# agent-charon/MinGraph-UNet

Hardware: AMD Instinct MI355X
Metric: segmented Mpix/sec, full MinGraph-UNet forward (U-Net + patch-graph GAT), 512x512 batch (higher is better)
Workload: dtype f32

## Files before the change

mingraph-unet_amd/csrc/common.h:

```cpp
#pragma once
#include <hip/hip_runtime.h>
#include <stdint.h>

namespace mgu {

struct Tuning {
  bool first_mfma = true;
  bool use_halo = true;
  bool halo_tps3 = true;
  int halo_max_ppb = 16;
  bool use_wino = true;
  int wino_mode = -1;
  int wino_prec = 1;
  bool wino_cp_narrow = true;
  bool wino_yfast = false;
  bool convt_frag = true;
  bool wino_deep = true;
  bool wino_cp = true;
  int wino_rounds = 1;
  int wino_ppb_cap = 32;
  bool wgrad_halo = true;
  bool wino_wgrad = true;
  bool convt_dgrad_x3 = true;
  bool wgrad_x3 = true;
  bool wgrad_thin = true;
  bool wino_dgrad = true;
  bool gat_fused = true;
  bool wino_ures = true;
  bool wino_prio = false;
  bool wino_asm_narrow = true;
  int wino_asm = 1;
};
const Tuning& default_tuning();
hipError_t ensure_dyn_lds(const void* func, size_t bytes, bool (&done)[64]);

struct IgemmDesc {
  const Tuning* tn;
  const float* in;
  const float* w;
  const float* wu;
  const float* scale;
  const float* shift;
  float* out;
  int M;
  int H, W;
  int Cp;
  int ldin;
  int KS;
  int K;
  int Kp;
  int N;
  int ldout;
  int coff;
  int relu;
  int out_mode;
  int ct_cout;
  int Hout, Wout;
  float* pool;
  int ldpool;
  double* stat_slots;
  int split_n;
  float* out2;
  int ld2;
};

inline const Tuning& tun(const IgemmDesc& d) { return d.tn ? *d.tn : default_tuning(); }
hipError_t launch_igemm_f32(const IgemmDesc& d, hipStream_t s);
int wino_grid_blocks(const IgemmDesc& d);
bool halo_pool_fusable(const IgemmDesc& d, int dtype);
hipError_t launch_igemm_bf16(const IgemmDesc& d, hipStream_t s);
const char* igemm_kernel_name(const IgemmDesc& d, int dtype);
size_t convt_x3_floats(int Cin, int Cout);
hipError_t launch_pack_convt_x3(const float* w, float* Wx, int Cin, int Cout, hipStream_t s);
bool convt_x3_applicable(const IgemmDesc& d);
hipError_t launch_convt_x3(const IgemmDesc& d, hipStream_t s);
size_t convt_bf16f_floats(int Cin, int Cout);
hipError_t launch_pack_convt_bf16f(const float* w, float* Wf, int Cin, int Cout, hipStream_t s);
bool convt_bf16f_applicable(const IgemmDesc& d);
hipError_t launch_convt_bf16f(const IgemmDesc& d, hipStream_t s);
size_t convt_x3_dgrad_floats(int Cin, int Cout);
hipError_t launch_pack_convt_x3_dgrad(const float* w, float* Wx, int Cin, int Cout, hipStream_t s);
bool convt_x3_dgrad_applicable(const IgemmDesc& d);
hipError_t launch_convt_x3_dgrad(const IgemmDesc& d, hipStream_t s);
hipError_t launch_pack_first_w(const float* w, float* wf, int Cout, int Cin, hipStream_t s);
size_t first_mfma_floats();
bool first_mfma_applicable(int dtype, int Cin, int Cp, int Cout, int ldout, int coff, int64_t H, int64_t W);
hipError_t launch_pack_first_mfma(const float* w, float* wfm, int Cout, int Cin, hipStream_t s);
hipError_t launch_first_mfma(int dtype, const void* in, const float* wfm, const float* scale, const float* shift, void* out, int B, int H,
                             int W, int ldout, int coff, int relu, hipStream_t s);
hipError_t launch_first_mfma_direct(int dtype, const float* x, int64_t sn, int64_t sc, int64_t sh, int64_t sw, int cin, const float* wfm,
                                    const float* scale, const float* shift, void* out, int B, int H, int W, int ldout, int coff, int relu,
                                    hipStream_t s);
bool first_conv_applicable(int dtype, int Cin, int Cp, int Cout, int ldout, int coff);
hipError_t launch_first_conv(int dtype, const void* in, const float* wf, const float* scale, const float* shift, void* out, int B, int H, int W,
                             int Cin, int Cout, int ldout, int coff, int relu, hipStream_t s);
size_t wino_u_floats(int Cout, int Cp);
hipError_t launch_pack_wino_w(const float* w, float* U, int Cout, int Cin, int Cp, int dgrad, int prec, hipStream_t s);
enum { PACK_WINO = 0, PACK_FIRST_W = 1, PACK_CONVT_X3 = 2, PACK_BIAS_TILE = 3, PACK_DGRAD_W = 4, PACK_FIRST_MFMA = 5 };
struct WinoPackItem {
  const float* w;
  float* U;
  int Cout, Cin, Cp, Np, dgrad;
  unsigned blk0;
  int kind;
  int reserved;
};
static_assert(sizeof(WinoPackItem) == 48, "WinoPackItem must have no padding");
constexpr int WINO_PACK_MAX = 64;
struct WinoPackBatch {
  int n, prec;
  unsigned total_blocks;
  WinoPackItem it[WINO_PACK_MAX];
};
bool wino_pack_batch_prepare(WinoPackBatch& b);
hipError_t launch_pack_wino_w_multi(const WinoPackBatch* batch_dev, unsigned total_blocks, hipStream_t s);
bool wino_applicable(const IgemmDesc& d);
hipError_t launch_wino_f32(const IgemmDesc& d, hipStream_t s);
bool wino_asm_applicable(const IgemmDesc& d);
hipError_t launch_wino_cp_asm(const IgemmDesc& d, hipStream_t s);

struct WgradDesc {
  const Tuning* tn;
  const float* z;
  int ldz, zoff;
  const float* in;
  int ldin, inoff, Cp;
  int KS;
  int M, H, W;
  int Hs, Ws;
  int N, K, Kp;
  float* dw;
  size_t dw_capacity;
  int groups;
  int rows_per_split;
};
inline const Tuning& tun(const WgradDesc& d) { return d.tn ? *d.tn : default_tuning(); }
hipError_t launch_wgrad_f32(WgradDesc& d, hipStream_t s);
bool wino_wgrad_applicable(const WgradDesc& d);
hipError_t launch_wino_wgrad_f32(WgradDesc& d, hipStream_t s);
bool wgrad_thin_applicable(const WgradDesc& d);
hipError_t launch_wgrad_thin(WgradDesc& d, hipStream_t s);

constexpr int STAT_ROWS = 576;
constexpr int CHAN_REDUCE_ROWS = 512;
size_t chan_reduce_work_bytes(int Cmax);
hipError_t launch_bn_stats(const float* z, int ldz, int64_t M, int C, double* work, double* sums, hipStream_t s);
hipError_t launch_bn_finalize(const double* sum, const double* sumsq, int64_t M, float eps, float momentum,
                              const float* gamma, const float* beta, float* mean, float* invstd, float* scale,
                              float* shift, float* run_mean, float* run_var, int C, hipStream_t s);
hipError_t launch_bn_finalize_slots(double* slots, int nrows, double* sums, int64_t M, float eps, float momentum, const float* gamma,
                                    const float* beta, float* mean, float* invstd, float* scale, float* shift, float* run_mean,
                                    float* run_var, int C, hipStream_t s);
hipError_t launch_bn_apply_relu(const float* z, const float* scale, const float* shift, float* y, int ldy, int64_t M, int C,
                                hipStream_t s);
hipError_t launch_bn_apply_relu_pool(const float* z, const float* scale, const float* shift, float* y, int ldy, float* pooled, int B, int H,
                                     int W, int C, hipStream_t s);
hipError_t launch_bn_bwd_reduce(const float* dy, int lddy, const float* fwd_scale, const float* fwd_shift, const float* z, int ldz,
                                const float* mean, const float* invstd, int64_t M, int C, double* work, double* sums,
                                float* dbeta, float* dgamma, hipStream_t s);
hipError_t launch_bn_bwd_apply(const float* dy, int lddy, const float* fwd_scale, const float* fwd_shift, const float* z, const float* mean,
                               const float* invstd, const float* gamma, const double* sums, int64_t M, int C, float* dz,
                               double* work, float* dbias, hipStream_t s);
hipError_t launch_bn_bwd_apply_deferred(const float* dy, int lddy, const float* fsc, const float* fsh, const float* z, const float* mean,
                                        const float* invstd, const float* gamma, const double* sums, int64_t M, int C, float* dz,
                                        double* work, int* rows, hipStream_t s);
hipError_t launch_colsum(const float* z, int ldz, int64_t M, int C, double* work, float* out, hipStream_t s);
hipError_t launch_maxpool2_bwd_add(const float* y, int ldy, const float* dpool, float* dskip, int ldd, int B, int H, int W,
                                   int C, hipStream_t s);
hipError_t launch_zero_pad_region(float* buf, int ld, int coff, int C, int B, int H, int W, int h2, int w2, hipStream_t s);
hipError_t launch_ce(const float* logits, const int64_t* labels, int64_t M, int C, long long ignore_index, float grad_scale,
                     float* dlogits, int ldd, double* acc, int* err_word, float* loss_out, hipStream_t s);
hipError_t launch_pack_dgrad_w(const float* w, float* wp, int Cout, int Cin, int Cop, int KS, int Kp, hipStream_t s);
hipError_t launch_pack_convt_dgrad_w(const float* w, float* wp, int Cin, int Cout, int Kp, hipStream_t s);
hipError_t launch_unpack_conv_grad(const float* dwp, int groups, size_t panel_stride, float* g, int Cout, int Cin, int Cp, int KS,
                                   int Kp, hipStream_t s, double* fold_slots = nullptr, int fold_rows = 0, int fold_n = 0, float* fold_out = nullptr);
hipError_t launch_unpack_convt_grad(const float* dwp, int groups, size_t panel_stride, float* g, int Cin, int Cout, int Kp, hipStream_t s);
hipError_t launch_sgd(float* p, const float* g, float* buf, int64_t n, float lr, float momentum, float wd, int step, float grad_scale,
                      hipStream_t s);
hipError_t launch_adam(float* p, const float* g, float* m, float* v, int64_t n, float lr, float b1, float b2, float eps,
                       float wd, int step, float grad_scale, hipStream_t s);

hipError_t launch_pack_input(const float* x, void* out, int dtype, int B, int C, int Cp, int H, int W, int64_t sn, int64_t sc,
                             int64_t sh, int64_t sw, hipStream_t s);
hipError_t launch_maxpool2(const void* in, int ldin, void* out, int dtype, int B, int H, int W, int C, hipStream_t s);
bool patch_mean_head_fusable(int dtype, int C, int ncls);
hipError_t launch_patch_mean(const void* feat, int dtype, float* out, int B, int H, int W, int C, int patch, hipStream_t s,
                             const float* head_w = nullptr, const float* head_b = nullptr, float* logits = nullptr, int ncls = 0);
hipError_t launch_pack_conv_w(const float* w_oihw, void* wp, int dtype, int Cout, int Cin, int Cp, int KS, int Kp, hipStream_t s);
hipError_t launch_pack_convt_w(const float* w_iohw, void* wp, int dtype, int Cin, int Cout, int Kp, hipStream_t s);
hipError_t launch_bn_fold(const float* bias, const float* gamma, const float* beta, const float* mean, const float* var,
                          float eps, float* scale, float* shift, int C, hipStream_t s);
hipError_t launch_bias_tile(const float* bias, float* shift, int C, int reps, hipStream_t s);
hipError_t launch_conv1x1_head(const void* in, int dtype, int ldin, int C, const float* w, const float* bias, float* out,
                               int ldout, int ncls, int64_t npix, hipStream_t s);
hipError_t launch_argmax(const float* logits, int64_t npix, int C, int64_t* pred, hipStream_t s);

hipError_t launch_gat_wa_rows(const float* W, const float* a, float* panel, int row0, int heads, int Fh, int Fin, int Kp, hipStream_t s);
bool gat_fused_applicable(int Fin, int heads, int Fh, int64_t E);
size_t gat_fused_scratch_floats(int Fin, int heads, int Fh);
hipError_t launch_gat_prep(const float* W, const float* a, float* wa, unsigned* Wx, int heads, int Fh, int Fin, hipStream_t s);
hipError_t launch_gat_stmax(const float* x, const float* wa, int N, int Fin, int heads, const int32_t* rowptr, const int32_t* col,
                            const int32_t* gp, int G, float alpha, float* st, int32_t* node_graph, unsigned long long* gmax, int gstride,
                            unsigned gen, hipStream_t s);
hipError_t launch_gat_fused(const float* x, int Fin, const float* st, const int32_t* rowptr, const int32_t* col, const int32_t* gp, int G,
                            const unsigned long long* gmax, const unsigned* Wx, int N, int heads, int Fh, int concat, float alpha, float* out,
                            int gstride, unsigned gen, hipStream_t s);
hipError_t launch_gat_node_graph(const int32_t* gp, int G, int nodes_per_graph, int N, int32_t* node_graph, hipStream_t s);
hipError_t launch_gat_edge_max(const float* st, const int32_t* rowptr, const int32_t* col, const int32_t* node_graph, int N,
                               int heads, float alpha, unsigned long long* gmax_enc, int gstride, unsigned gen, hipStream_t s);
hipError_t launch_gat_aggregate(const float* wh, int P, const float* st, const int32_t* rowptr, const int32_t* col,
                                const int32_t* node_graph, const unsigned long long* gmax_enc, int N, int64_t E, int heads, int Fh,
                                int concat, float alpha, float* out, int gstride, unsigned gen, hipStream_t s);

}
```

mingraph-unet_amd/csrc/convt_x3.hip:

```cpp
#include <hip/hip_runtime.h>
#include <stdint.h>

#include <algorithm>
#include <type_traits>

#include "common.h"
#include "pack_small.h"

namespace mgu {

typedef float f32x16 __attribute__((ext_vector_type(16)));
typedef float f32x4 __attribute__((ext_vector_type(4)));
typedef unsigned u32x4 __attribute__((ext_vector_type(4)));
typedef __bf16 bf16x8 __attribute__((ext_vector_type(8)));

namespace {

__device__ __forceinline__ void split3_pack(const float a, const float b, unsigned& p0, unsigned& p1, unsigned& p2) {
  const unsigned ua = __float_as_uint(a), ub = __float_as_uint(b);
  p0 = __builtin_amdgcn_perm(ub, ua, 0x07060302u);
  const float ra = a - __uint_as_float(ua & 0xffff0000u), rb = b - __uint_as_float(ub & 0xffff0000u);
  const unsigned va = __float_as_uint(ra), vb = __float_as_uint(rb);
  p1 = __builtin_amdgcn_perm(vb, va, 0x07060302u);
  const float sa = ra - __uint_as_float(va & 0xffff0000u), sb = rb - __uint_as_float(vb & 0xffff0000u);
  p2 = __builtin_amdgcn_perm(__float_as_uint(sb), __float_as_uint(sa), 0x07060302u);
}

__device__ __forceinline__ f32x16 mfma_bf16(const u32x4 a, const u32x4 b, const f32x16 c) {
  return __builtin_amdgcn_mfma_f32_32x32x16_bf16(__builtin_bit_cast(bf16x8, a), __builtin_bit_cast(bf16x8, b), c, 0, 0, 0);
}

__global__ void pack_convt_x3_kernel(const float* __restrict__ w, uint16_t* __restrict__ Wx, int Cin, int Cout) {
  pack_convt_x3_body(w, Wx, Cin, Cout, 0, blockIdx.x, gridDim.x);
}

__device__ __forceinline__ void lds_barrier() { asm volatile("s_waitcnt lgkmcnt(0)\n\ts_barrier" ::: "memory"); }

template <int MODE, int NI>
__global__ __launch_bounds__(256, 2) void convt2x2_x3_kernel(const float* __restrict__ in, const int ldin, const uint16_t* __restrict__ Wx,
                                                             const float* __restrict__ shift, float* __restrict__ out, const int M,
                                                             const int H, const int W, const int Cin, const int Cout, const int ldout,
                                                             const int coff, const int Hout, const int Wout, const int ntn,
                                                             const int nblocks) {
  constexpr int AP = 40, ABUF = 3 * 128 * AP;
  __shared__ __attribute__((aligned(16))) uint16_t As[2 * ABUF];
  __shared__ int rowoff[128];
  const int chunk = gridDim.x >> 3;
  const int lb = (blockIdx.x & 7) * chunk + (blockIdx.x >> 3);
  if (lb >= nblocks) return;
  const int nt = lb % ntn, mt = lb / ntn;
  const int tid = threadIdx.x, lane = tid & 63, wave = tid >> 6;
  const int wm = wave >> 1, wn = wave & 1, lr = lane & 31, lh = lane >> 5;
  const int bm0 = mt * 128;
  const int HW = H * W;
  long long pix0;
  {
    const int img = bm0 / HW, rem = bm0 - img * HW, y = rem / W;
    pix0 = ((long long)img * Hout + 2 * y) * Wout + 2 * (rem - y * W);
  }
  if (tid < 128) {
    const int m = bm0 + tid;
    int off = 0;
    if (m < M) {
      const int img = m / HW, rem = m - img * HW, y = rem / W, x = rem - y * W;
      off = (int)((((long long)img * Hout + 2 * y) * Wout + 2 * x - pix0) * ldout);
    }
    rowoff[tid] = off;
  }

  const int arow = tid >> 3, ach = (tid & 7) * 4;
  const float* aptr[4];
#pragma unroll
  for (int j = 0; j < 4; ++j) {
    const int m = min(bm0 + j * 32 + arow, M - 1);
    if (MODE == 0) {
      aptr[j] = in + (size_t)m * ldin + ach;
    } else {
      const int img = m / HW, rem = m - img * HW, y = rem / W, x = rem - y * W;
      aptr[j] = in + (((size_t)img * Hout + 2 * y) * Wout + 2 * x) * ldin + ach;
    }
  }
  const int nk = (MODE == 0 ? Cin : 4 * Cin) >> 5;
  const int spq = Cin >> 5;
  auto koff = [&](int s) -> int {
    if (MODE == 0) return s * 32;
    const int q = s / spq;
    return ((q >> 1) * Wout + (q & 1)) * ldin + (s - q * spq) * 32;
  };
  f32x4 areg[2][4];
  auto load_a = [&](int s, auto set_t) {
    constexpr int set = decltype(set_t)::value;
    const int ko = koff(s);
#pragma unroll
    for (int j = 0; j < 4; ++j) areg[set][j] = *reinterpret_cast<const f32x4*>(aptr[j] + ko);
  };
  auto store_a = [&](int buf, auto set_t) {
    constexpr int set = decltype(set_t)::value;
    uint16_t* const base = As + buf * ABUF + arow * AP + ach;
#pragma unroll
    for (int j = 0; j < 4; ++j) {
      unsigned p[3][2];
      split3_pack(areg[set][j][0], areg[set][j][1], p[0][0], p[1][0], p[2][0]);
      split3_pack(areg[set][j][2], areg[set][j][3], p[0][1], p[1][1], p[2][1]);
#pragma unroll
      for (int q = 0; q < 3; ++q) *reinterpret_cast<uint2*>(base + (q * 128 + j * 32) * AP) = uint2{p[q][0], p[q][1]};
    }
  };

  const int nt128 = NI == 2 ? nt : nt >> 1, sub0 = NI == 2 ? wn * 2 : (nt & 1) * 2 + wn;
  const u32x4* const bp = reinterpret_cast<const u32x4*>(Wx) + ((size_t)nt128 * (2 * nk) * 12 + sub0 * 3) * 64 + lane;
  u32x4 br[2][3 * NI];
  auto load_b = [&](int kk, auto buf_t) {
    constexpr int buf = decltype(buf_t)::value;
#pragma unroll
    for (int f = 0; f < 3 * NI; ++f) br[buf][f] = bp[((size_t)kk * 12 + f) * 64];
  };

  f32x16 acc[2][NI];
#pragma unroll
  for (int mi = 0; mi < 2; ++mi)
#pragma unroll
    for (int ni = 0; ni < NI; ++ni)
#pragma unroll
      for (int r = 0; r < 16; ++r) acc[mi][ni][r] = 0.f;

  const int aoff = (wm * 64 + lr) * AP + lh * 8;
  auto half_step = [&](int buf, int ss, auto bb_t) {
    constexpr int bb = decltype(bb_t)::value;
    u32x4 pa[2][3];
#pragma unroll
    for (int mi = 0; mi < 2; ++mi)
#pragma unroll
      for (int q = 0; q < 3; ++q)
        pa[mi][q] = *reinterpret_cast<const u32x4*>(As + buf * ABUF + (q * 128 + mi * 32) * AP + aoff + ss * 16);
#pragma unroll
    for (int mi = 0; mi < 2; ++mi)
#pragma unroll
      for (int ni = 0; ni < NI; ++ni) {
        f32x16 t = acc[mi][ni];
        t = mfma_bf16(pa[mi][2], br[bb][ni * 3 + 0], t);
        t = mfma_bf16(pa[mi][0], br[bb][ni * 3 + 2], t);
        t = mfma_bf16(pa[mi][1], br[bb][ni * 3 + 1], t);
        t = mfma_bf16(pa[mi][1], br[bb][ni * 3 + 0], t);
        t = mfma_bf16(pa[mi][0], br[bb][ni * 3 + 1], t);
        t = mfma_bf16(pa[mi][0], br[bb][ni * 3 + 0], t);
        acc[mi][ni] = t;
      }
  };
  using B0 = std::integral_constant<int, 0>;
  using B1 = std::integral_constant<int, 1>;
  const int nkk = 2 * nk;
  load_a(0, B0{});
  load_a(min(1, nk - 1), B1{});
  load_b(0, B0{});
  store_a(0, B0{});
  lds_barrier();
  auto second_half_and_stage = [&](int buf, auto bb_t, auto set_t) {
    half_step(buf, 1, bb_t);
    store_a(buf ^ 1, set_t);
#pragma unroll
    for (int k = 0; k < 12 * NI; ++k) {
      __builtin_amdgcn_sched_group_barrier(0x008, 1, 0);
      __builtin_amdgcn_sched_group_barrier(0x002, NI == 2 ? 4 : 8, 0);
    }
    __builtin_amdgcn_sched_group_barrier(0x200, 12, 0);
  };
  for (int s = 0; s < nk; s += 2) {
    load_a(min(s + 2, nk - 1), B0{});
    load_b(min(2 * s + 1, nkk - 1), B1{});
    __builtin_amdgcn_sched_barrier(0);
    half_step(0, 0, B0{});
    load_b(min(2 * s + 2, nkk - 1), B0{});
    __builtin_amdgcn_sched_barrier(0);
    second_half_and_stage(0, B1{}, B1{});
    __builtin_amdgcn_sched_barrier(0);
    lds_barrier();
    if (s + 1 >= nk) break;
    load_a(min(s + 3, nk - 1), B1{});
    load_b(min(2 * s + 3, nkk - 1), B1{});
    __builtin_amdgcn_sched_barrier(0);
    half_step(1, 0, B0{});
    load_b(min(2 * s + 4, nkk - 1), B0{});
    __builtin_amdgcn_sched_barrier(0);
    second_half_and_stage(1, B1{}, B0{});
    __builtin_amdgcn_sched_barrier(0);
    lds_barrier();
  }

  float* const tile_out = MODE == 0 ? out + (size_t)pix0 * ldout + coff : out + (size_t)bm0 * ldout + coff;
  const bool full_m = bm0 + 128 <= M;
  auto store_tile = [&](auto guarded_t) {
    constexpr bool GUARDED = decltype(guarded_t)::value;
#pragma unroll
    for (int ni = 0; ni < NI; ++ni) {
      const int n = nt * (64 * NI) + wn * (32 * NI) + ni * 32 + lr;
      int ncol = n;
      if (MODE == 0) {
        const int q = n / Cout;
        ncol = ((q >> 1) * Wout + (q & 1)) * ldout + (n - q * Cout);
      }
      const float sh = shift ? shift[n] : 0.f;
#pragma unroll
      for (int mi = 0; mi < 2; ++mi)
#pragma unroll
        for (int r = 0; r < 16; ++r) {
          const int rrow = wm * 64 + mi * 32 + (r & 3) + 8 * (r >> 2) + 4 * lh;
          const unsigned idx = (unsigned)((MODE == 0 ? rowoff[rrow] : rrow * ldout) + ncol);
          const float v = acc[mi][ni][r] + sh;
          if (!GUARDED) tile_out[idx] = v;
          else if (bm0 + rrow < M) tile_out[idx] = v;
        }
    }
  };
#if defined(MGU_DIAG) && MGU_DIAG == 7
  {
    float sacc = 0.f;
#pragma unroll
    for (int mi = 0; mi < 2; ++mi)
#pragma unroll
      for (int ni = 0; ni < NI; ++ni)
#pragma unroll
        for (int r = 0; r < 16; ++r) sacc += acc[mi][ni][r];
    if (sacc == 123.456f) tile_out[tid] = sacc;
  }
#else
  if (full_m) store_tile(std::false_type{});
  else store_tile(std::true_type{});
#endif
}

}

size_t convt_x3_floats(int Cin, int Cout) { return (size_t)Cin * Cout * 6; }


namespace {

__global__ void pack_convt_x3_dgrad_kernel(const float* __restrict__ w, uint16_t* __restrict__ Wx, int Cin, int Cout) {
  pack_convt_x3_body(w, Wx, Cin, Cout, 1, blockIdx.x, gridDim.x);
}

}

size_t convt_x3_dgrad_floats(int Cin, int Cout) { return (size_t)((Cin + 127) / 128 * 128) * Cout * 6; }

hipError_t launch_pack_convt_x3_dgrad(const float* w, float* Wx, int Cin, int Cout, hipStream_t s) {
  if ((Cin & 63) || (Cout & 31)) return hipErrorInvalidValue;
  hipLaunchKernelGGL(pack_convt_x3_dgrad_kernel, dim3((unsigned)std::min<int64_t>(4096, ((int64_t)Cin * Cout * 4 + 255) / 256)), dim3(256), 0, s, w,
                     reinterpret_cast<uint16_t*>(Wx), Cin, Cout);
  return hipGetLastError();
}

bool convt_x3_dgrad_applicable(const IgemmDesc& d) {
  return d.KS == 2 && d.wu && d.out_mode == 0 && (d.Cp & 31) == 0 && d.K == 4 * d.Cp && (d.N & 63) == 0 && (d.ldin & 3) == 0 && !d.scale &&
         !d.shift && !d.relu && !d.split_n && !d.pool && tun(d).wino_prec != 0 && (long)d.M * d.ldout < (1l << 31) &&
         (long)d.Hout * d.Wout * d.ldin < (1l << 31);
}

hipError_t launch_convt_x3_dgrad(const IgemmDesc& d, hipStream_t s) {
  const bool wide = (d.N & 127) == 0;
  const int mtiles = (d.M + 127) / 128, ntn = d.N / (wide ? 128 : 64);
  const int nb = mtiles * ntn;
  const int chunk = (nb + 7) / 8;
  if (wide)
    hipLaunchKernelGGL((convt2x2_x3_kernel<1, 2>), dim3(chunk * 8), dim3(256), 0, s, d.in, d.ldin, reinterpret_cast<const uint16_t*>(d.wu),
                       (const float*)nullptr, d.out, d.M, d.H, d.W, d.Cp, d.N, d.ldout, d.coff, d.Hout, d.Wout, ntn, nb);
  else
    hipLaunchKernelGGL((convt2x2_x3_kernel<1, 1>), dim3(chunk * 8), dim3(256), 0, s, d.in, d.ldin, reinterpret_cast<const uint16_t*>(d.wu),
                       (const float*)nullptr, d.out, d.M, d.H, d.W, d.Cp, d.N, d.ldout, d.coff, d.Hout, d.Wout, ntn, nb);
  return hipGetLastError();
}

hipError_t launch_pack_convt_x3(const float* w, float* Wx, int Cin, int Cout, hipStream_t s) {
  if ((Cin & 15) || (Cout & 31)) return hipErrorInvalidValue;
  hipLaunchKernelGGL(pack_convt_x3_kernel, dim3((unsigned)std::min<int64_t>(4096, ((int64_t)Cin * Cout * 4 + 255) / 256)), dim3(256), 0, s, w, reinterpret_cast<uint16_t*>(Wx), Cin,
                     Cout);
  return hipGetLastError();
}

bool convt_x3_applicable(const IgemmDesc& d) {
  return d.out_mode == 1 && d.wu && d.KS == 1 && d.K == d.Cp && (d.Cp & 31) == 0 && (d.ct_cout & 31) == 0 && d.N == 4 * d.ct_cout &&
         (d.ldin & 3) == 0 && !d.scale && !d.relu && !d.split_n && tun(d).wino_prec != 0 &&
         (9l * 128 + 8l * d.Wout) * d.ldout < (1l << 31);
}

hipError_t launch_convt_x3(const IgemmDesc& d, hipStream_t s) {
  const int mtiles = (d.M + 127) / 128, ntn = d.N / 128;
  const int nb = mtiles * ntn;
  const int chunk = (nb + 7) / 8;
  hipLaunchKernelGGL((convt2x2_x3_kernel<0, 2>), dim3(chunk * 8), dim3(256), 0, s, d.in, d.ldin, reinterpret_cast<const uint16_t*>(d.wu), d.shift, d.out,
                     d.M, d.H, d.W, d.Cp, d.ct_cout, d.ldout, d.coff, d.Hout, d.Wout, ntn, nb);
  return hipGetLastError();
}

}
```

mingraph-unet_amd/csrc/mgunet_api.hip:

```cpp
#include "ctx.h"

#include <algorithm>

using namespace mgu;
using namespace mgud;

namespace mgud {
std::string g_create_err;
}

namespace {

struct WsPlan {
  size_t xin, tmp, bott, total;
  std::vector<size_t> pooled;
};

WsPlan plan_ws(const mgu_ctx* c, int B, int H, int W) {
  std::vector<int> hs, wsz;
  level_dims(H, W, c->depth, hs, wsz);
  WsPlan p;
  size_t off = 0;
  const size_t es = c->dtype == MGU_DTYPE_BF16 ? 2 : 4;
  auto take = [&](size_t elems) {
    size_t o = off;
    off += (elems * es + 255) / 256 * 256;
    return o;
  };
  p.xin = take((size_t)B * H * W * c->Cp0);
  size_t tmax = 0;
  for (int i = 0; i <= c->depth; ++i) {
    size_t f = (size_t)B * hs[i] * wsz[i] * ((size_t)c->feat << i);
    if (f > tmax) tmax = f;
  }
  p.tmp = take(tmax);
  for (int i = 0; i < c->depth; ++i) p.pooled.push_back(take((size_t)B * hs[i + 1] * wsz[i + 1] * ((size_t)c->feat << i)));
  p.bott = take((size_t)B * hs[c->depth] * wsz[c->depth] * ((size_t)c->feat << c->depth));
  p.total = off;
  return p;
}

}

extern "C" {

const char* mgu_version(void) { return "mgunet 0.2 (gfx950: fp32 Winograd / bf16 MFMA forward, fp32 training step, GAT, RCCL gradient exchange)"; }

int mgu_create(int device_id, mgu_ctx** out) {
  if (!out) return fail(nullptr, MGU_ERR_INVALID, "out == NULL");
  int n = 0;
  hipError_t e = hipGetDeviceCount(&n);
  if (e != hipSuccess || n <= 0)
    return fail(nullptr, MGU_ERR_HIP, "no HIP device available (%s): libmgunet has no CPU fallback",
                e != hipSuccess ? hipGetErrorString(e) : "device count 0");
  if (device_id < 0 || device_id >= n) return fail(nullptr, MGU_ERR_INVALID, "device %d out of range [0,%d)", device_id, n);
  e = hipSetDevice(device_id);
  if (e != hipSuccess) return fail(nullptr, MGU_ERR_HIP, "hipSetDevice: %s", hipGetErrorString(e));
  mgu_ctx* c = new mgu_ctx();
  c->device = device_id;
  auto flag = [](const char* name) { const char* v = getenv(name); return v && v[0] == '1'; };
  auto num = [](const char* name, int dflt) { const char* v = getenv(name); return v && v[0] ? atoi(v) : dflt; };
  Tuning& t = c->tn;
  t.first_mfma = !flag("MGU_NO_FIRST_MFMA");
  t.use_halo = !flag("MGU_NO_HALO");
  t.halo_tps3 = !flag("MGU_HALO_TPS1");
  t.halo_max_ppb = std::max(1, num("MGU_HALO_PPB", t.halo_max_ppb));
  t.use_wino = !flag("MGU_NO_WINOGRAD");
  t.wino_mode = num("MGU_WINO_MODE", -1);
  t.wino_prec = num("MGU_WINO_PREC", t.wino_prec) ? 1 : 0;
  t.wino_cp = !flag("MGU_NO_WINO_CP");
  t.wino_deep = !flag("MGU_NO_WINO_DEEP");
  t.convt_frag = !flag("MGU_NO_CONVT_FRAG");
  t.wino_yfast = flag("MGU_WINO_YFAST");
  t.wino_cp_narrow = num("MGU_WINO_CP_NARROW", 1) != 0;
  t.wino_rounds = std::max(1, num("MGU_WINO_ROUNDS", 1));
  t.wino_ppb_cap = std::max(1, num("MGU_WINO_PPB_CAP", 32));
  t.wgrad_halo = !flag("MGU_NO_WGRAD_HALO");
  t.wino_wgrad = !flag("MGU_NO_WINO_WGRAD");
  t.wgrad_x3 = !flag("MGU_NO_WGRAD_X3");
  t.convt_dgrad_x3 = !flag("MGU_NO_CONVT_DGRAD_X3");
  t.wgrad_thin = !flag("MGU_NO_THIN_WGRAD");
  t.wino_dgrad = !flag("MGU_NO_WINO_DGRAD");
  t.gat_fused = !flag("MGU_NO_GAT_FUSED");
  t.wino_ures = !flag("MGU_NO_WINO_URES");
  t.wino_prio = flag("MGU_WINO_PRIO");
  t.wino_asm = std::max(0, num("MGU_WINO_ASM", t.wino_asm));
  t.wino_asm_narrow = num("MGU_WINO_ASM_NARROW", 1) != 0;
  *out = c;
  return MGU_OK;
}

void mgu_destroy(mgu_ctx* c) {
  if (!c) return;
  (void)hipSetDevice(c->device);
  (void)hipDeviceSynchronize();
  (void)mgu_comm_destroy(c);
  if (c->arena) (void)hipFree(c->arena);
  if (c->ws) (void)hipFree(c->ws);
  if (c->gws) (void)hipFree(c->gws);
  if (c->gbws) (void)hipFree(c->gbws);
  if (c->pack_dev) (void)hipFree(c->pack_dev);
  if (c->gbpanel) (void)hipFree(c->gbpanel);
  if (c->tws) (void)hipFree(c->tws);
  if (c->redws) (void)hipFree(c->redws);
  if (c->wuws) (void)hipFree(c->wuws);
  if (c->ncws) (void)hipFree(c->ncws);
  if (c->lossws) (void)hipFree(c->lossws);
  if (c->imgws) (void)hipFree(c->imgws);
  gat_destroy(c);
  if (c->err_word) (void)hipHostFree(c->err_word);
  for (auto e : c->ev) (void)hipEventDestroy(e);
  for (auto e : c->ev_total)
    if (e) (void)hipEventDestroy(e);
  delete c;
}

const char* mgu_last_error(mgu_ctx* c) { return c ? c->err.c_str() : g_create_err.c_str(); }

int mgu_unet_configure(mgu_ctx* c, int in_ch, int ncls, int feat, int depth, int dtype) {
  if (!c) return MGU_ERR_INVALID;
  if (in_ch < 1 || ncls < 1 || feat < 4 || (feat & 3) || depth < 1 || depth > 8)
    return fail(c, MGU_ERR_INVALID, "unsupported UNet(%d,%d,%d,%d): init_features must be a positive multiple of 4, depth 1..8",
                in_ch, ncls, feat, depth);
  if (dtype != MGU_DTYPE_F32 && dtype != MGU_DTYPE_BF16) return fail(c, MGU_ERR_INVALID, "unknown dtype %d", dtype);
  if (dtype == MGU_DTYPE_BF16 && ((feat & 7) || ncls > 4))
    return fail(c, MGU_ERR_INVALID, "bf16 storage needs init_features %% 8 == 0 (16-byte lanes of 8 bf16) and <= 4 classes");
  HIPCHK(c, hipSetDevice(c->device));
  c->in_ch = in_ch, c->ncls = ncls, c->feat = feat, c->depth = depth, c->dtype = dtype;
  c->Cp0 = rup(in_ch, dtype == MGU_DTYPE_BF16 ? 8 : 4);
  c->layers.clear();
  auto add_block = [&](const std::string& prefix, int cin, int cp, int cout) {
    for (int j = 0; j < 2; ++j) {
      Layer L;
      L.prefix = prefix;
      L.conv = j == 0 ? "conv1" : "conv2";
      L.bn = j == 0 ? "bn1" : "bn2";
      L.Cin = j == 0 ? cin : cout;
      L.Cp = j == 0 ? cp : cout;
      L.Cout = cout;
      L.KS = 3;
      c->layers.push_back(L);
    }
  };
  int cin = in_ch, cp = c->Cp0, f = feat;
  for (int i = 0; i < depth; ++i) {
    add_block("encoder.encoder_blocks." + std::to_string(i) + ".", cin, cp, f);
    cin = cp = f;
    f *= 2;
  }
  add_block("encoder.bottleneck.", cin, cp, f);
  int prev = f;
  for (int b = 0; b < depth; ++b) {
    const int ci = feat << (depth - 1 - b);
    Layer U;
    U.prefix = "decoder.decoder_blocks." + std::to_string(b) + ".";
    U.conv = "upsample";
    U.Cin = U.Cp = prev;
    U.Cout = prev / 2;
    U.KS = 1;
    U.convt = true;
    c->layers.push_back(U);
    add_block(U.prefix + "conv_block.", ci + prev / 2, ci + prev / 2, ci);
    prev = ci;
  }
  Layer Fc;
  Fc.prefix = "decoder.";
  Fc.conv = "final_conv";
  Fc.Cin = Fc.Cp = prev;
  Fc.Cout = ncls;
  Fc.KS = 1;
  c->layers.push_back(Fc);

  size_t total = 0;
  for (auto& L : c->layers) {
    L.K = L.KS * L.KS * L.Cp;
    L.Kp = rup(L.K, dtype == MGU_DTYPE_BF16 ? 64 : 32);
    L.N = L.convt ? 4 * L.Cout : L.Cout;
    L.Np = rup(L.N, 128);
    total += (size_t)L.Np * L.Kp + 2 * (size_t)L.Np + (L.bn.empty() ? 0 : 4 * (size_t)L.Np);
    L.wino = dtype == MGU_DTYPE_F32 && !L.convt && L.KS == 3 && L.Cp % 16 == 0;
    if (L.wino) total += wino_u_floats(L.Cout, L.Cp);
    if (L.wino && rup(L.Cout, 4) % 16 == 0) total += wino_u_floats(L.Cin, rup(L.Cout, 4));
    L.ctx3 = dtype == MGU_DTYPE_F32 && L.convt && L.Cin % 32 == 0 && L.Cout % 32 == 0 && c->tn.wino_prec != 0 && c->tn.convt_frag;
    if (L.ctx3) total += convt_x3_floats(L.Cin, L.Cout) + convt_x3_dgrad_floats(L.Cin, L.Cout);
    L.ctb = dtype == MGU_DTYPE_BF16 && L.convt && L.Cin % 64 == 0 && L.Cout % 32 == 0 && c->tn.convt_frag;
    if (L.ctb) total += convt_bf16f_floats(L.Cin, L.Cout);
    if (dtype == MGU_DTYPE_F32 && !L.convt && L.bn.empty()) total += (size_t)rup(L.Cin, 128) * rup(L.KS * L.KS * rup(L.Cout, 4), 32);
    L.first = !L.convt && L.KS == 3 && first_conv_applicable(dtype, L.Cin, L.Cp, L.Cout, 8, 0);
    if (L.first) total += 9 * 4 * (size_t)L.Cout + first_mfma_floats();
  }
  {
    int64_t off = 0;
    size_t i = 0;
    auto wsize = [](const Layer& L) { return (int64_t)L.Cout * L.Cin * L.KS * L.KS * (L.convt ? 4 : 1); };
    while (i < c->layers.size()) {
      Layer& A = c->layers[i];
      if (!A.bn.empty()) {
        Layer& B2 = c->layers[i + 1];
        A.off_w = off, off += wsize(A);
        A.off_b = off, off += A.Cout;
        B2.off_w = off, off += wsize(B2);
        B2.off_b = off, off += B2.Cout;
        A.off_gamma = off, off += A.Cout;
        A.off_beta = off, off += A.Cout;
        B2.off_gamma = off, off += B2.Cout;
        B2.off_beta = off, off += B2.Cout;
        i += 2;
      } else {
        A.off_w = off, off += wsize(A);
        A.off_b = off, off += A.Cout;
        i += 1;
      }
    }
    c->nparams = off;
  }
  if (c->arena) HIPCHK(c, hipFree(c->arena));
  c->arena = nullptr;
  HIPCHK(c, hipMalloc((void**)&c->arena, total * sizeof(float)));
  HIPCHK(c, hipMemset(c->arena, 0, total * sizeof(float)));
  c->arena_floats = total;
  float* p = c->arena;
  for (auto& L : c->layers) {
    L.wp = p;
    p += (size_t)L.Np * L.Kp;
    L.scale = p;
    p += L.Np;
    L.shift = p;
    p += L.Np;
    L.wu = nullptr;
    if (L.wino) L.wu = p, p += wino_u_floats(L.Cout, L.Cp);
    L.wug = nullptr, L.wug_valid = false;
    if (L.wino && rup(L.Cout, 4) % 16 == 0) L.wug = p, p += wino_u_floats(L.Cin, rup(L.Cout, 4));
    if (L.ctx3) L.wu = p, p += convt_x3_floats(L.Cin, L.Cout);
    if (L.ctb) L.wu = p, p += convt_bf16f_floats(L.Cin, L.Cout);
    L.wxg = nullptr, L.wxg_valid = false;
    if (L.ctx3) L.wxg = p, p += convt_x3_dgrad_floats(L.Cin, L.Cout);
    if (c->dtype == MGU_DTYPE_F32 && !L.convt && L.bn.empty()) L.wxg = p, p += (size_t)rup(L.Cin, 128) * rup(L.KS * L.KS * rup(L.Cout, 4), 32);
    L.wf = nullptr;
    if (L.first) L.wf = p, p += 9 * 4 * (size_t)L.Cout;
    L.wfm = nullptr;
    if (L.first) L.wfm = p, p += first_mfma_floats();
    if (!L.bn.empty()) {
      L.mean = p, p += L.Np;
      L.invstd = p, p += L.Np;
      L.tscale = p, p += L.Np;
      L.tshift = p, p += L.Np;
    }
  }
  c->configured = true;
  c->have_train_fwd = false;
  c->loaded = false;
  return MGU_OK;
}

int64_t mgu_unet_param_count(mgu_ctx* c) {
  if (!c || !c->configured) return -1;
  return c->nparams;
}

int64_t mgu_unet_param_offset(mgu_ctx* c, const char* name) {
  if (!c || !c->configured || !name) return -1;
  const std::string key(name);
  for (auto& L : c->layers) {
    if (key == L.prefix + L.conv + ".weight") return L.off_w;
    if (key == L.prefix + L.conv + ".bias") return L.off_b;
    if (!L.bn.empty()) {
      if (key == L.prefix + L.bn + ".weight") return L.off_gamma;
      if (key == L.prefix + L.bn + ".bias") return L.off_beta;
    }
  }
  return -1;
}

int mgu_unet_load_weights(mgu_ctx* c, const mgu_tensor_desc* named, int n, void* hip_stream) {
  if (!c) return MGU_ERR_INVALID;
  if (!c->configured) return fail(c, MGU_ERR_STATE, "mgu_unet_configure must precede mgu_unet_load_weights");
  if (!named || n <= 0) return fail(c, MGU_ERR_INVALID, "empty state_dict");
  HIPCHK(c, hipSetDevice(c->device));
  hipStream_t s = (hipStream_t)hip_stream;
  std::map<std::string, const mgu_tensor_desc*> sd;
  for (int i = 0; i < n; ++i)
    if (named[i].name) sd[named[i].name] = &named[i];
  auto get = [&](const std::string& key, int64_t numel, const float** out) -> int {
    auto it = sd.find(key);
    if (it == sd.end()) return fail(c, MGU_ERR_INVALID, "state_dict is missing key '%s'", key.c_str());
    if (it->second->numel != numel)
      return fail(c, MGU_ERR_INVALID, "state_dict key '%s' has %lld elements, expected %lld", key.c_str(),
                  (long long)it->second->numel, (long long)numel);
    if (!it->second->ptr) return fail(c, MGU_ERR_INVALID, "state_dict key '%s' has a NULL pointer", key.c_str());
    *out = (const float*)it->second->ptr;
    return MGU_OK;
  };
  for (auto& L : c->layers) {
    const float *w, *b;
    const std::string cw = L.prefix + L.conv;
    int rc;
    if (L.convt) {
      if ((rc = get(cw + ".weight", (int64_t)L.Cin * L.Cout * 4, &w))) return rc;
      if ((rc = get(cw + ".bias", L.Cout, &b))) return rc;
      L.w_src = w, L.b_src = b;
    } else {
      if ((rc = get(cw + ".weight", (int64_t)L.Cout * L.Cin * L.KS * L.KS, &w))) return rc;
      if ((rc = get(cw + ".bias", L.Cout, &b))) return rc;
      L.w_src = w, L.b_src = b;
      if (!L.bn.empty()) {
        const float *g, *be, *rm, *rv;
        const std::string bn = L.prefix + L.bn;
        if ((rc = get(bn + ".weight", L.Cout, &g))) return rc;
        if ((rc = get(bn + ".bias", L.Cout, &be))) return rc;
        if ((rc = get(bn + ".running_mean", L.Cout, &rm))) return rc;
        if ((rc = get(bn + ".running_var", L.Cout, &rv))) return rc;
        L.gamma = g, L.beta = be, L.run_mean = const_cast<float*>(rm), L.run_var = const_cast<float*>(rv);
      }
    }
  }
  int rc = repack_weights(c, s);
  if (rc) return rc;
  c->loaded = true;
  return MGU_OK;
}

int mgu_unet_refresh_weights(mgu_ctx* c, void* hip_stream) {
  if (!c) return MGU_ERR_INVALID;
  if (!c->configured || !c->loaded) return fail(c, MGU_ERR_STATE, "mgu_unet_refresh_weights needs a preceding mgu_unet_load_weights");
  HIPCHK(c, hipSetDevice(c->device));
  return repack_weights(c, (hipStream_t)hip_stream);
}

int mgu_unet_workspace_bytes(mgu_ctx* c, int B, int H, int W, int training, size_t* out) {
  if (!c || !out) return MGU_ERR_INVALID;
  if (!c->configured) return fail(c, MGU_ERR_STATE, "not configured");
  *out = training ? train_ws_bytes(c, B, H, W) : plan_ws(c, B, H, W).total;
  return MGU_OK;
}

int mgu_unet_reserve(mgu_ctx* c, int B, int H, int W, int training) {
  size_t need = 0;
  int rc = mgu_unet_workspace_bytes(c, B, H, W, training, &need);
  if (rc) return rc;
  HIPCHK(c, hipSetDevice(c->device));
  return training ? ensure(c, &c->tws, &c->tws_bytes, need) : ensure(c, &c->ws, &c->ws_bytes, need);
}

}

int mgud::repack_weights(mgu_ctx* c, hipStream_t s) {
  std::vector<WinoPackItem> items;
  for (auto& L : c->layers) {
    const float *w = L.w_src, *b = L.b_src;
    L.wxg_valid = false;
    if (L.convt) {
      L.wp_dirty = L.ctx3;
      if (!L.ctx3) HIPCHK(c, launch_pack_convt_w(w, L.wp, c->dtype, L.Cin, L.Cout, L.Kp, s));
      if (L.ctb) HIPCHK(c, launch_pack_convt_bf16f(w, L.wu, L.Cin, L.Cout, s));
      if (L.ctx3) items.push_back(WinoPackItem{w, L.wu, L.Cout, L.Cin, 0, 0, 0, 0, PACK_CONVT_X3});
      items.push_back(WinoPackItem{b, L.shift, L.Cout, 4, 0, 0, 0, 0, PACK_BIAS_TILE});
      if (L.wxg && c->want_train && c->tn.convt_dgrad_x3 && (L.Cin & 63) == 0 && (L.Cout & 31) == 0) {
        items.push_back(WinoPackItem{w, L.wxg, L.Cout, L.Cin, 0, 0, 1, 0, PACK_CONVT_X3});
        L.wxg_valid = true;
      }
    } else {
      L.wp_dirty = true;
      if (L.wu) items.push_back(WinoPackItem{w, L.wu, L.Cout, L.Cin, L.Cp, 0, 0, 0, PACK_WINO});
      L.wug_valid = false;
      if (L.wug && c->want_train && c->tn.wino_dgrad && c->tn.use_wino) {
        items.push_back(WinoPackItem{w, L.wug, L.Cin, L.Cout, rup(L.Cout, 4), 0, 1, 0, PACK_WINO});
        L.wug_valid = true;
      }
      const bool head_kernel = L.bn.empty() && c->ncls <= 4;
      if (!L.wu && !L.first && !head_kernel) {
        HIPCHK(c, launch_pack_conv_w(w, L.wp, c->dtype, L.Cout, L.Cin, L.Cp, L.KS, L.Kp, s));
        L.wp_dirty = false;
      }
      if (L.wf) items.push_back(WinoPackItem{w, L.wf, L.Cout, L.Cin, 0, 0, 0, 0, PACK_FIRST_W});
      if (L.wfm && L.Cout == 32 && L.Cin <= 3) items.push_back(WinoPackItem{w, L.wfm, L.Cout, L.Cin, 0, 0, 0, 0, PACK_FIRST_MFMA});
// ... 539 lines not shown
```

Baseline: 777.2.

## Add persistent transposed-conv x3 kernel overlapping tile epilogue with next prologue

Adds a persistent variant of the 2x2 transposed-convolution split-bf16 GEMM kernel. Grid size is capped at the resident workgroup count, and each workgroup loops over tiles. While one tile's results are stored, the next tile's A/B loads and row offsets are already in flight, using double-buffered row offset tables. This targets launch and tail overhead plus the idle epilogue gap, at the cost of more register pressure, a fixed occupancy of 2, and a static per-device cache of the resident count. It is enabled by default only when Cin/32 is even.

```diff
diff --git a/mingraph-unet_amd/csrc/common.h b/mingraph-unet_amd/csrc/common.h
--- a/mingraph-unet_amd/csrc/common.h
+++ b/mingraph-unet_amd/csrc/common.h
@@ -15,6 +15,7 @@
   bool wino_cp_narrow = true;
   bool wino_yfast = false;
   bool convt_frag = true;
+  bool convt_persist = true;
   bool wino_deep = true;
   bool wino_cp = true;
   int wino_rounds = 1;
diff --git a/mingraph-unet_amd/csrc/convt_x3.hip b/mingraph-unet_amd/csrc/convt_x3.hip
--- a/mingraph-unet_amd/csrc/convt_x3.hip
+++ b/mingraph-unet_amd/csrc/convt_x3.hip
@@ -2,6 +2,7 @@
 #include <stdint.h>
 
 #include <algorithm>
+#include <atomic>
 #include <type_traits>
 
 #include "common.h"
@@ -229,6 +230,219 @@
 #endif
 }
 
+__global__ __launch_bounds__(256, 2) void convt2x2_x3p_kernel(const float* __restrict__ in, const int ldin, const uint16_t* __restrict__ Wx,
+                                                              const float* __restrict__ shift, float* __restrict__ out, const int M,
+                                                              const int H, const int W, const int Cin, const int Cout, const int ldout,
+                                                              const int coff, const int Hout, const int Wout, const int ntn,
+                                                              const int nitems) {
+  constexpr int AP = 40, ABUF = 3 * 128 * AP;
+  __shared__ __attribute__((aligned(16))) uint16_t As[2 * ABUF];
+  __shared__ int rowoff[2][128];
+  const int g = gridDim.x >> 3, chunk = (nitems + 7) >> 3;
+  const int item_end = min(((int)blockIdx.x & 7) * chunk + chunk, nitems);
+  int li = ((int)blockIdx.x & 7) * chunk + ((int)blockIdx.x >> 3);
+  if (li >= item_end) return;
+  const int tid = threadIdx.x, lane = tid & 63, wave = tid >> 6;
+  const int wm = wave >> 1, wn = wave & 1, lr = lane & 31, lh = lane >> 5;
+  const int HW = H * W;
+  const int arow = tid >> 3, ach = (tid & 7) * 4;
+  const int nk = Cin >> 5, nkk = 2 * nk;
+
+  auto tile_of = [&](int item, int& bm0, int& nt, long long& pix0) {
+    nt = item % ntn;
+    bm0 = (item / ntn) * 128;
+    const int img = bm0 / HW, rem = bm0 - img * HW, y = rem / W;
+    pix0 = ((long long)img * Hout + 2 * y) * Wout + 2 * (rem - y * W);
+  };
+  const float* aptr[4];
+  const u32x4* bp;
+  auto setup = [&](int item, int rb) {
+    int bm0, nt;
+    long long pix0;
+    tile_of(item, bm0, nt, pix0);
+    if (tid < 128) {
+      const int m = bm0 + tid;
+      int off = 0;
+      if (m < M) {
+        const int mimg = m / HW, mrem = m - mimg * HW, my = mrem / W, mx = mrem - my * W;
+        off = (int)((((long long)mimg * Hout + 2 * my) * Wout + 2 * mx - pix0) * ldout);
+      }
+      rowoff[rb][tid] = off;
+    }
+#pragma unroll
+    for (int j = 0; j < 4; ++j) aptr[j] = in + (size_t)min(bm0 + j * 32 + arow, M - 1) * ldin + ach;
+    bp = reinterpret_cast<const u32x4*>(Wx) + ((size_t)nt * (2 * nk) * 12 + wn * 6) * 64 + lane;
+  };
+
+  f32x4 areg[2][4];
+  auto load_a = [&](int s, auto set_t) {
+    constexpr int set = decltype(set_t)::value;
+#pragma unroll
+    for (int j = 0; j < 4; ++j) areg[set][j] = *reinterpret_cast<const f32x4*>(aptr[j] + s * 32);
+  };
+  auto store_a = [&](int buf, auto set_t) {
+    constexpr int set = decltype(set_t)::value;
+    uint16_t* const base = As + buf * ABUF + arow * AP + ach;
+#pragma unroll
+    for (int j = 0; j < 4; ++j) {
+      unsigned p[3][2];
+      split3_pack(areg[set][j][0], areg[set][j][1], p[0][0], p[1][0], p[2][0]);
+      split3_pack(areg[set][j][2], areg[set][j][3], p[0][1], p[1][1], p[2][1]);
+#pragma unroll
+      for (int q = 0; q < 3; ++q) *reinterpret_cast<uint2*>(base + (q * 128 + j * 32) * AP) = uint2{p[q][0], p[q][1]};
+    }
+  };
+  u32x4 br[2][6];
+  auto load_b = [&](int kk, auto buf_t) {
+    constexpr int buf = decltype(buf_t)::value;
+#pragma unroll
+    for (int f = 0; f < 6; ++f) br[buf][f] = bp[((size_t)kk * 12 + f) * 64];
+  };
+  f32x16 acc[2][2];
+  const int aoff = (wm * 64 + lr) * AP + lh * 8;
+  auto half_step = [&](int buf, int ss, auto bb_t) {
+    constexpr int bb = decltype(bb_t)::value;
+    u32x4 pa[2][3];
+#pragma unroll
+    for (int mi = 0; mi < 2; ++mi)
+#pragma unroll
+      for (int q = 0; q < 3; ++q)
+        pa[mi][q] = *reinterpret_cast<const u32x4*>(As + buf * ABUF + (q * 128 + mi * 32) * AP + aoff + ss * 16);
+#pragma unroll
+    for (int mi = 0; mi < 2; ++mi)
+#pragma unroll
+      for (int ni = 0; ni < 2; ++ni) {
+        f32x16 t = acc[mi][ni];
+        t = mfma_bf16(pa[mi][2], br[bb][ni * 3 + 0], t);
+        t = mfma_bf16(pa[mi][0], br[bb][ni * 3 + 2], t);
+        t = mfma_bf16(pa[mi][1], br[bb][ni * 3 + 1], t);
+        t = mfma_bf16(pa[mi][1], br[bb][ni * 3 + 0], t);
+        t = mfma_bf16(pa[mi][0], br[bb][ni * 3 + 1], t);
+        t = mfma_bf16(pa[mi][0], br[bb][ni * 3 + 0], t);
+        acc[mi][ni] = t;
+      }
+  };
+  using B0 = std::integral_constant<int, 0>;
+  using B1 = std::integral_constant<int, 1>;
+  auto second_half_and_stage = [&](int buf, auto bb_t, auto set_t) {
+    half_step(buf, 1, bb_t);
+    store_a(buf ^ 1, set_t);
+#pragma unroll
+    for (int k = 0; k < 24; ++k) {
+      __builtin_amdgcn_sched_group_barrier(0x008, 1, 0);
+      __builtin_amdgcn_sched_group_barrier(0x002, 4, 0);
+    }
+    __builtin_amdgcn_sched_group_barrier(0x200, 12, 0);
+  };
+
+  int rb = 0;
+  setup(li, rb);
+  load_a(0, B0{});
+  load_a(min(1, nk - 1), B1{});
+  load_b(0, B0{});
+  store_a(0, B0{});
+  lds_barrier();
+  for (;;) {
+#pragma unroll
+    for (int mi = 0; mi < 2; ++mi)
+#pragma unroll
+      for (int ni = 0; ni < 2; ++ni)
+#pragma unroll
+        for (int r = 0; r < 16; ++r) acc[mi][ni][r] = 0.f;
+    for (int s = 0; s < nk; s += 2) {
+      load_a(min(s + 2, nk - 1), B0{});
+      load_b(min(2 * s + 1, nkk - 1), B1{});
+      __builtin_amdgcn_sched_barrier(0);
+      half_step(0, 0, B0{});
+      load_b(min(2 * s + 2, nkk - 1), B0{});
+      __builtin_amdgcn_sched_barrier(0);
+      second_half_and_stage(0, B1{}, B1{});
+      __builtin_amdgcn_sched_barrier(0);
+      lds_barrier();
+     
+      load_a(min(s + 3, nk - 1), B1{});
+      load_b(min(2 * s + 3, nkk - 1), B1{});
+      __builtin_amdgcn_sched_barrier(0);
+      half_step(1, 0, B0{});
+      load_b(min(2 * s + 4, nkk - 1), B0{});
+      __builtin_amdgcn_sched_barrier(0);
+      second_half_and_stage(1, B1{}, B0{});
+      __builtin_amdgcn_sched_barrier(0);
+      lds_barrier();
+    }
+    int etid = tid;
+    asm volatile("" : "+v"(etid));
+    const int ewm = etid >> 7, ewn = (etid >> 6) & 1, elr = etid & 31, elh = (etid >> 5) & 1;
+    int cbm0, cnt;
+    long long cpix0;
+    tile_of(li, cbm0, cnt, cpix0);
+    float sh[2];
+#pragma unroll
+    for (int ni = 0; ni < 2; ++ni) sh[ni] = shift ? shift[cnt * 128 + ewn * 64 + ni * 32 + elr] : 0.f;
+    const int crb = rb;
+    const int next = li + g;
+    const bool more = next < item_end;
+    rb ^= 1;
+    setup(more ? next : li, rb);
+    load_a(0, B0{});
+    load_a(min(1, nk - 1), B1{});
+    load_b(0, B0{});
+    __builtin_amdgcn_sched_barrier(0);
+    float* const tile_out = out + (size_t)cpix0 * ldout + coff;
+    auto store_tile = [&](auto guarded_t) {
+      constexpr bool GUARDED = decltype(guarded_t)::value;
+#pragma unroll
+      for (int ni = 0; ni < 2; ++ni) {
+        const int n = cnt * 128 + ewn * 64 + ni * 32 + elr;
+        const int q = n / Cout;
+        const int ncol = ((q >> 1) * Wout + (q & 1)) * ldout + (n - q * Cout);
+#pragma unroll
+        for (int mi = 0; mi < 2; ++mi)
+#pragma unroll
+          for (int r = 0; r < 16; ++r) {
+            const int rrow = ewm * 64 + mi * 32 + (r & 3) + 8 * (r >> 2) + 4 * elh;
+            const unsigned idx = (unsigned)(rowoff[crb][rrow] + ncol);
+            const float v = acc[mi][ni][r] + sh[ni];
+            if (!GUARDED) __builtin_nontemporal_store(v, tile_out + idx);
+            else if (cbm0 + rrow < M) __builtin_nontemporal_store(v, tile_out + idx);
+          }
+      }
+    };
+#if defined(MGU_DIAG) && MGU_DIAG == 7
+    {
+      float sacc = 0.f;
+#pragma unroll
+      for (int mi = 0; mi < 2; ++mi)
+#pragma unroll
+        for (int ni = 0; ni < 2; ++ni)
+#pragma unroll
+          for (int r = 0; r < 16; ++r) sacc += acc[mi][ni][r];
+      if (sacc == 123.456f) tile_out[tid] = sacc;
+    }
+    if (!more) break;
+    __builtin_amdgcn_sched_barrier(0);
+    store_a(0, B0{});
+    lds_barrier();
+#else
+    auto stage_next = [&]() {
+      __builtin_amdgcn_sched_barrier(0);
+      store_a(0, B0{});
+      lds_barrier();
+    };
+    if (cbm0 + 128 <= M) {
+      store_tile(std::false_type{});
+      if (!more) break;
+      stage_next();
+    } else {
+      store_tile(std::true_type{});
+      if (!more) break;
+      stage_next();
+    }
+#endif
+    li = next;
+  }
+}
+
 }
 
 size_t convt_x3_floats(int Cin, int Cout) { return (size_t)Cin * Cout * 6; }
@@ -287,6 +501,25 @@
 hipError_t launch_convt_x3(const IgemmDesc& d, hipStream_t s) {
   const int mtiles = (d.M + 127) / 128, ntn = d.N / 128;
   const int nb = mtiles * ntn;
+  if (tun(d).convt_persist && ((d.Cp >> 5) & 1) == 0) {
+    static std::atomic<int> resident_of[64];
+    int dev = 0;
+    (void)hipGetDevice(&dev);
+    std::atomic<int>& slot = resident_of[dev >= 0 && dev < 64 ? dev : 0];
+    int resident = slot.load(std::memory_order_relaxed);
+    if (!resident) {
+      int cus = 256, occ = 2;
+      (void)hipDeviceGetAttribute(&cus, hipDeviceAttributeMultiprocessorCount, dev);
+      if (hipOccupancyMaxActiveBlocksPerMultiprocessor(&occ, reinterpret_cast<const void*>(&convt2x2_x3p_kernel), 256, 0) != hipSuccess || occ < 1)
+        occ = 2;
+      resident = std::max(8, cus * occ / 8 * 8);
+      slot.store(resident, std::memory_order_relaxed);
+    }
+    const int nwg = std::min((nb + 7) / 8 * 8, resident);
+    hipLaunchKernelGGL(convt2x2_x3p_kernel, dim3(nwg), dim3(256), 0, s, d.in, d.ldin, reinterpret_cast<const uint16_t*>(d.wu), d.shift, d.out,
+                       d.M, d.H, d.W, d.Cp, d.ct_cout, d.ldout, d.coff, d.Hout, d.Wout, ntn, nb);
+    return hipGetLastError();
+  }
   const int chunk = (nb + 7) / 8;
   hipLaunchKernelGGL((convt2x2_x3_kernel<0, 2>), dim3(chunk * 8), dim3(256), 0, s, d.in, d.ldin, reinterpret_cast<const uint16_t*>(d.wu), d.shift, d.out,
                      d.M, d.H, d.W, d.Cp, d.ct_cout, d.ldout, d.coff, d.Hout, d.Wout, ntn, nb);
diff --git a/mingraph-unet_amd/csrc/mgunet_api.hip b/mingraph-unet_amd/csrc/mgunet_api.hip
--- a/mingraph-unet_amd/csrc/mgunet_api.hip
+++ b/mingraph-unet_amd/csrc/mgunet_api.hip
@@ -71,6 +71,7 @@
   t.wino_cp = !flag("MGU_NO_WINO_CP");
   t.wino_deep = !flag("MGU_NO_WINO_DEEP");
   t.convt_frag = !flag("MGU_NO_CONVT_FRAG");
+  t.convt_persist = !flag("MGU_NO_CONVT_PERSIST");
   t.wino_yfast = flag("MGU_WINO_YFAST");
   t.wino_cp_narrow = num("MGU_WINO_CP_NARROW", 1) != 0;
   t.wino_rounds = std::max(1, num("MGU_WINO_ROUNDS", 1));
```

Result: no change. 777.2, median of 6 (-0.0%).
